# maxgillett/tinysplat

Hardware: AMD Instinct MI355X
Metric: Gaussians*pixels/s fwd+bwd (higher is better)
Workload: dtype f32; 1 GPU; 1000000 random Gaussians, SH degree 3, 1920x1080, fwd+bwd (RGB), BASELINE configs[2]; max_per_tile=614, parallelism=single GPU, tile_lists=16x16 (gsplat's) (auto), gaussian_order=as generated (i.i.d.)

## Files before the change

### include/tinysplat_hip.h

```cpp
#ifndef TINYSPLAT_HIP_H
#define TINYSPLAT_HIP_H

#include <stdint.h>

#ifdef __cplusplus
extern "C" {
#endif

#define TS_ABI_VERSION 8

#define TS_E_BADARG (-1)
#define TS_E_DEGREE (-2)

#define TS_TILE 16
#define TS_SPLAT_RECORD_FLOATS 12
#define TS_PARTIAL_ROW_FLOATS 12

int ts_abi_version(void);

typedef struct ts_camera {
    float fx, fy, cx, cy;
    int32_t img_width, img_height;
    int32_t tile_bounds_x, tile_bounds_y;
    int32_t tile_row0, tile_rows;
// ... 118 lines not shown
#define TS_RASTER_NARROW_WAVES 8
#define TS_RASTER_FLAG_GEN(g) (((g) & 0xff) << 8)
int ts_raster_fwd(int32_t channels, int32_t flags, const ts_camera* cam_host, const int32_t* tile_bins,
                  const int32_t* gaussian_ids_sorted, const float* splats, const float* background,
                  float* out_img, float* final_Ts, int32_t* final_index, uint8_t* clamp_mask,
                  void* stream);
int ts_raster_fwd_planes(int32_t channels, int32_t flags, const ts_camera* cam_host, const int32_t* tile_bins,
                         const int32_t* gaussian_ids_sorted, const float* splats, const float* background,
                         float* out_img, float* out_depth, float* final_Ts, int32_t* final_index,
                         uint8_t* clamp_mask, void* stream);

int ts_raster_fwd_sort(int32_t channels, int32_t flags, const ts_camera* cam_host, const int32_t* tile_bins,
                       const int32_t* bucket_ids, const float* depths, int32_t* gaussian_ids_sorted,
                       const float* splats, const float* background, float* out_img, float* out_depth,
                       float* final_Ts, int32_t* final_index, uint8_t* clamp_mask, void* stream);

int ts_raster_bwd(int32_t channels, int32_t flags, int64_t num_intersects, const ts_camera* cam_host,
                  const int32_t* tile_bins, const int32_t* gaussian_ids_sorted, const float* splats,
                  const float* background, const float* final_Ts, const int32_t* final_index,
                  const float* v_out_img, const float* v_out_alpha, const uint8_t* clamp_mask,
                  float* partials, uint8_t* row_flags, void* stream);
int ts_raster_bwd_planes(int32_t channels, int32_t flags, int64_t num_intersects, const ts_camera* cam_host,
                         const int32_t* tile_bins, const int32_t* gaussian_ids_sorted, const float* splats,
                         const float* background, const float* final_Ts, const int32_t* final_index,
                         const float* v_out_img, const float* v_out_depth, int32_t planes,
                         const float* v_out_alpha, const uint8_t* clamp_mask,
                         float* partials, uint8_t* row_flags, void* stream);

int ts_reduce_partials(int32_t n, int32_t channels, int32_t flags, const int32_t* num_tiles_hit,
                       const int32_t* cum_tiles_hit, const float* partials,
                       const uint8_t* row_flags, const float* splats, float* v_xy, float* v_conic,
                       float* v_colors, float* v_opacity, float* v_depth, const uint8_t* color_mask,
                       void* stream);

#define TS_FRAME_TIGHT 1
#define TS_FRAME_SPLIT 2
#define TS_FRAME_NARROW_WAVES 8
#define TS_FRAME_DIRECT_SCATTER 32
#define TS_FRAME_PLANES 64
#define TS_FRAME_LIST_STATS 256
#define TS_FRAME_SEPARATE_SORT 128
#define TS_FRAME_STRIPE 16
#define TS_FRAME_GROUP_COUNTS 1024
#define TS_FRAME_ONE_WALK 2048
#define TS_FRAME_ROW_SPANS (4096)
#define TS_FRAME_SURVIVORS 512
typedef struct ts_frame {
    int32_t n, num_bases, sh_degree, channels, flags;
    int32_t flag_gen;
    ts_camera cam;
    const float *means, *scales, *quats, *opacities, *colors_dc, *colors_rest;
    const float *view34, *projview, *origin, *background;
    float *xys, *depths, *conics, *colors, *splats;
    int32_t *radii, *num_tiles_hit, *cum_tiles_hit;
    uint8_t* sh_mask;
    int32_t *scan_ws, *bin_ws, *tile_bins;
    int32_t* total_host;
    int64_t num_intersects;
    int64_t capacity;
    int32_t *bucket_ids, *gaussian_ids_sorted;
    float *out_img, *final_Ts;
    int32_t* final_index;
    uint8_t* clamp_mask;
    const float* v_out_img;
    float* partials;
    uint8_t* row_flags;
// ... 361 lines not shown
```

### tinysplat_amd/_lib.py

```python
from __future__ import annotations

import ctypes
import os
from ctypes import POINTER, c_double, c_float, c_int32, c_int64, c_uint32, c_uint64, c_void_p
from pathlib import Path

LIB_PATH = Path(os.environ["TS_LIB_PATH"]) if os.environ.get("TS_LIB_PATH") else \
    Path(__file__).resolve().parent / "csrc" / "libtinysplat_hip.so"
ABI_VERSION = 8
HINT_BALANCED_WALK = 1
HINT_COOP_SPLIT = 1 << 20
RASTER_LOGIT_OPACITY = 1
RASTER_CLAMP_RGB = 2
RASTER_SPLIT_BLOCKS = 4
RASTER_NARROW_WAVES = 8
FRAME_TIGHT = 1
FRAME_SPLIT = 2
FRAME_NARROW_WAVES = 8
FRAME_STRIPE = 16
FRAME_DIRECT_SCATTER = 32
FRAME_PLANES = 64
FRAME_SEPARATE_SORT = 128
FRAME_LIST_STATS = 256
FRAME_SURVIVORS = 512
# ... 114 lines not shown
    "ts_colors_pack_fwd": (c_int32, [c_int32, c_int32, c_int32, _P, _P, _P, _P, _P, _P, c_int32, c_int32,
                                     _P, _P, _P, _P, _P, _CAM, _P, _P, _P]),
    "ts_colors_pack_spans_fwd": (c_int32, [c_int32, c_int32, c_int32, _P, _P, _P, _P, _P, _P, c_int32, c_int32,
                                           _P, _P, _P, _P, _P, _CAM, _P, _P, c_int32, _P, _P]),
    "ts_pack_splats": (c_int32, [c_int32, c_int32, c_int32, _P, _P, _P, _P, _P, _P, _CAM, _P, _P, _P]),
    "ts_raster_fwd": (c_int32, [c_int32, c_int32, _CAM, _P, _P, _P, _P, _P, _P, _P, _P, _P]),
    "ts_raster_bwd": (c_int32, [c_int32, c_int32, c_int64, _CAM, _P, _P, _P, _P, _P, _P, _P, _P, _P, _P, _P, _P]),
    "ts_raster_fwd_planes": (c_int32, [c_int32, c_int32, _CAM, _P, _P, _P, _P, _P, _P, _P, _P, _P, _P]),
    "ts_raster_fwd_sort": (c_int32, [c_int32, c_int32, _CAM, _P, _P, _P, _P, _P, _P, _P, _P, _P, _P, _P, _P]),
    "ts_raster_bwd_planes": (c_int32, [c_int32, c_int32, c_int64, _CAM, _P, _P, _P, _P, _P, _P, _P, _P, c_int32,
                                       _P, _P, _P, _P, _P]),
    "ts_bench_stream_read": (c_int32, [_P, c_int64, _P, _P]),
    "ts_bench_gather48": (c_int32, [_P, _P, c_int64, _P, _P]),
    "ts_photometric_ws_floats": (c_int64, [c_int32, c_int32]),
    "ts_photometric_loss": (c_int32, [c_int32, c_int32, _P, _P, c_float, c_float, _P, _P, _P]),
    "ts_photometric_loss_rgbd": (c_int32, [c_int32, c_int32, c_int32, _P, _P, _P, c_float, c_float, c_float, _P, _P, _P]),
    "ts_photometric_loss_planes": (c_int32, [c_int32, c_int32, _P, _P, _P, _P, c_float, c_float, c_float, _P, _P, _P,
                                             _P]),
    "ts_photometric_loss_reduce": (c_int32, [c_int32, c_int32, c_float, c_float, c_float, _P, _P, _P]),
    "ts_adam_step": (c_int32, [c_int32, _P, _P, _P, _P, _P, _P, _P, c_float, c_float, c_float, _P]),
    "ts_sh_colors_bwd_adam": (c_int32, [c_int32, c_int32, c_int32, _P, _P, _P, _P, _P, _P, _ADAM, _P]),
    "ts_project_bwd_adam": (c_int32, [c_int32, _P, _P, _P, _P, _P, _CAM, c_int32, _P, _P, _P, _P, _P, _P, _ADAM, _P]),
    "ts_frame_bwd_params_adam": (c_int32, [_FRAME, _ADAM, _P]),
    "ts_grad_accum": (c_int32, [c_int32, _P, _P, _P]),
    "ts_densify_classify": (c_int32, [c_int32, _P, _P, _P, POINTER(TsDensifyPolicy), _P, _P]),
    "ts_densify_ws_ints": (c_int64, [c_int32]),
    "ts_densify_plan": (c_int32, [c_int32, _P, _P, _P, _P, _P]),
    "ts_gather_rows": (c_int32, [c_int32, _P, _P, _P, c_int32, c_int32, _P, _P]),
    "ts_split_fixup": (c_int32, [c_int32, _P, _P, _P, _P, _P, _P, _P, _P]),
    "ts_ply_row_floats": (c_int32, [c_int32]),
    "ts_ply_pack_rows": (c_int32, [c_int32, c_int32, _P, _P, _P, _P, _P, _P, _P, _P]),
    "ts_ply_unpack_rows": (c_int32, [c_int32, c_int32, _P, _P, _P, _P, _P, _P, _P, _P]),
    "ts_reduce_partials": (c_int32, [c_int32, c_int32, c_int32, _P, _P, _P, _P, _P, _P, _P, _P, _P, _P, _P, _P]),
    "ts_route_ws_ints": (c_int64, [c_int32, c_int32]),
    "ts_route_count": (c_int32, [c_int32, _P, _P, _CAM, _STRIPES, _P, _P, _P]),
    "ts_route_count_padded": (c_int32, [c_int32, _P, _P, _CAM, _STRIPES, _P, _P, _P, _P]),
    "ts_route_pack": (c_int32, [c_int32, c_int32, _P, _P, _P, _P, _CAM, _STRIPES, _P, _P, _P]),
    "ts_import_records": (c_int32, [c_int32, _P, _CAM, _P, _P, _P, _P, _P]),
    "ts_import_pack": (c_int32, [c_int32, _P, _P, _CAM, _P, _P]),
    "ts_reduce_partials_rows": (c_int32, [c_int32, c_int32, c_int32, _P, _P, _P, _P, _P, _P, _P]),
    "ts_route_accumulate": (c_int32, [c_int32, c_int32, _P, _P, _P, _P, _CAM, _STRIPES, _P, _P, _P, _P, _P, _P, _P, _P]),
    "ts_shard_owner_fwd": (c_int32, [_FRAME, _STRIPES, _P, _P, _P]),
    "ts_shard_owner_fwd_padded": (c_int32, [_FRAME, _STRIPES, _P, _P, _P, _P]),
    "ts_shard_owner_fwd_fused": (c_int32, [c_int32, c_int32, c_int32, _P, _P, _P, _P, _P, _CAM, c_int32, _P, _P, _P, _P,
                                           c_int32, c_int32, _P, _P, _P, _P, _P, _P, _P, _STRIPES, _P, _P, _P, _P]),
    "ts_shard_owner_bwd_fused": (c_int32, [c_int32, c_int32, c_int32, c_int32, _P, _P, _P, _P, _P, _P, _P, _P, _P, _P,
                                           _CAM, _STRIPES, _P, _P, _P, _P, _P, _P, _P, _P, _P, _P, _P, _P, _P]),
    "ts_shard_stripe_fwd_import": (c_int32, [_FRAME, _P, _P]),
    "ts_shard_stripe_bwd": (c_int32, [_FRAME, _P, _P]),
    "ts_shard_owner_bwd": (c_int32, [_FRAME, _STRIPES, _P, _P, _P]),
    "ts_rank_step_struct_bytes": (c_int32, []),
    "ts_shard_rank_fwd_a": (c_int32, [_FRAME, _RANK, _P]),
    "ts_shard_rank_fwd_b": (c_int32, [_FRAME, _RANK, _P]),
    "ts_shard_rank_bwd_a": (c_int32, [_FRAME, _RANK, _P]),
    "ts_shard_rank_bwd_b": (c_int32, [_FRAME, _RANK, _P]),
    "ts_frame_struct_bytes": (c_int32, []),
    "ts_frame_fwd_project": (c_int32, [_FRAME, _P]),
    "ts_frame_fwd_prepare": (c_int32, [_FRAME, _P]),
    "ts_frame_fwd_composite": (c_int32, [_FRAME, _P]),
    "ts_frame_bwd_composite": (c_int32, [_FRAME, _P]),
    "ts_frame_bwd_params": (c_int32, [_FRAME, _P]),
    "ts_set_entry_probe": (c_int32, [_P, _P]),
    "ts_knn_ws_bytes": (c_int64, [c_int32, c_int32, c_int32]),
    "ts_knn": (c_int32, [c_int32, _P, c_int32, _P, c_int32, _P, _P, _P, _P, _P]),
    "ts_init_from_points": (c_int32, [c_int32, c_int32, _P, _P, _P, _P, _P, _P, _P, _P, _P, _P, _P, _P, _P, _P]),
    "ts_opacity_entropy_ws_bytes": (c_int64, [c_int32]),
# ... 129 lines not shown
```

### tinysplat_amd/csrc/frame.hip

```cpp
#include <hip/hip_runtime.h>

#include <atomic>
#include <cstdlib>
#if !defined(TS_NO_ROCTX) && __has_include(<rocprofiler-sdk-roctx/roctx.h>)
#include <rocprofiler-sdk-roctx/roctx.h>
#define TS_HAVE_ROCTX 1
#else
#define TS_HAVE_ROCTX 0
#endif

#include "../../include/tinysplat_hip.h"
#include "raster_survivors.h"

struct TsRange {
#if TS_HAVE_ROCTX
    explicit TsRange(const char* name) { roctxRangePush(name); }
    ~TsRange() { roctxRangePop(); }
#else
    explicit TsRange(const char*) {}
#endif
};

static std::atomic<ts_entry_probe> g_probe{nullptr};
static std::atomic<void*> g_probe_user{nullptr};
// ... 194 lines not shown
                            ts_sort_tiles_stats(num_tiles(f), f->tile_bins, f->depths, f->bucket_ids,
                                                f->gaussian_ids_sorted, f->bin_ws, counter, f->n, f->bin_ws, longest,
                                                stream)));
    }
    if (fused_sort)
        return TS_ENTRY("ts_raster_fwd",
                        ts_surv::raster_fwd_sort(f->channels, raster_flags(f), &f->cam, f->tile_bins, f->bucket_ids,
                                                 f->depths, f->gaussian_ids_sorted, f->splats, f->background,
                                                 f->out_img, planes ? f->out_depth : nullptr, f->final_Ts,
                                                 f->final_index, f->clamp_mask, survivors(f) ? f->survivors : nullptr,
                                                 stream));
    return TS_ENTRY("ts_raster_fwd",
                    ts_raster_fwd_planes(f->channels, raster_flags(f), &f->cam, f->tile_bins, f->gaussian_ids_sorted,
                                         f->splats, f->background, f->out_img, planes ? f->out_depth : nullptr,
                                         f->final_Ts, f->final_index, f->clamp_mask, stream));
}

int ts_frame_bwd_composite(const ts_frame* f, void* stream) {
    TsRange range_("ts_frame_bwd_composite");
    if (bad(f) || f->num_intersects < 0) return TS_E_BADARG;
    const bool planes = (f->flags & TS_FRAME_PLANES) != 0;
    const bool surv = survivors(f);
    TS_TRY(TS_ENTRY("ts_raster_bwd",
                    ts_surv::raster_bwd(f->channels,
                                        ((raster_flags(f) & ~(TS_RASTER_CLAMP_RGB | TS_RASTER_SPLIT_BLOCKS)) | bwd_split(f)) |
                                            TS_RASTER_FLAG_GEN(f->flag_gen),
                                        f->num_intersects, &f->cam, f->tile_bins, f->gaussian_ids_sorted, f->splats,
                                        f->background, f->final_Ts, f->final_index, f->v_out_img,
                                        planes ? f->v_out_depth : nullptr, planes ? 1 : 0, nullptr, f->clamp_mask,
                                        f->partials, f->row_flags, surv ? f->bucket_ids : nullptr,
                                        surv ? f->survivors : nullptr, stream)));
    const bool stripe = (f->flags & TS_FRAME_STRIPE) != 0;
    return TS_ENTRY("ts_reduce_partials",
                    ts_reduce_partials(f->n, f->channels,
                                       TS_RASTER_LOGIT_OPACITY | bwd_split(f) | TS_RASTER_FLAG_GEN(f->flag_gen),
                                       f->num_tiles_hit, f->cum_tiles_hit, f->partials, f->row_flags, f->splats,
                                       f->v_xy, f->v_conic, f->v_colors, f->v_opacity,
                                       f->channels == 4 ? f->v_depth : nullptr, stripe ? f->sh_mask : nullptr, stream));
}

int ts_frame_bwd_params(const ts_frame* f, void* stream) {
    TsRange range_("ts_frame_bwd_params");
    if (bad(f)) return TS_E_BADARG;
    TS_TRY(TS_ENTRY("ts_sh_colors_bwd",
                    ts_sh_colors_bwd(f->n, f->sh_degree, f->num_bases, f->means, f->origin,
                                     (f->flags & TS_FRAME_STRIPE) ? nullptr : f->sh_mask, f->v_colors, f->v_colors_dc,
                                     f->num_bases > 1 ? f->v_colors_rest : nullptr, stream)));
    return TS_ENTRY("ts_project_bwd",
                    ts_project_bwd(f->n, f->means, f->scales, f->quats, f->view34, f->projview, &f->cam, 3, f->radii,
                                   f->v_xy, f->v_depth, f->v_conic, nullptr, f->v_means, f->v_scales, f->v_quats,
                                   stream));
}

int ts_frame_bwd_params_adam(const ts_frame* f, const ts_adam* adam, void* stream) {
    TsRange range_("ts_frame_bwd_params_adam");
    if (bad(f) || !adam) return TS_E_BADARG;
    TS_TRY(TS_ENTRY("ts_sh_colors_bwd_adam",
                    ts_sh_colors_bwd_adam(f->n, f->sh_degree, f->num_bases, f->means, f->origin,
                                          (f->flags & TS_FRAME_STRIPE) ? nullptr : f->sh_mask, f->v_colors,
                                          const_cast<float*>(f->colors_dc),
                                          f->num_bases > 1 ? const_cast<float*>(f->colors_rest) : nullptr, adam,
                                          stream)));
    return TS_ENTRY("ts_project_bwd_adam",
                    ts_project_bwd_adam(f->n, const_cast<float*>(f->means), const_cast<float*>(f->scales),
                                        const_cast<float*>(f->quats), f->view34, f->projview, &f->cam, 3, f->radii,
                                        f->v_xy, f->v_depth, f->v_conic, const_cast<float*>(f->opacities), f->v_opacity,
                                        adam, stream));
}


int ts_shard_owner_fwd(const ts_frame* fo, const ts_stripes* stripes, int32_t* route_ws, int32_t* counts,
// ... 132 lines not shown
```

### tinysplat_amd/csrc/pack.h

```cpp
#pragma once

#include <hip/hip_runtime.h>

#include "../../include/tinysplat_hip.h"
#include "row_spans.h"
#include "splat_math.h"

namespace ts {

struct PackArgs {
    int channels, flags;
    const float* xys;
    const int* radii;
    const float* conics;
    const float* opacity;
    const int* cum_tiles_hit;
    const float* depths;
    float4* splats;
    ts_camera cam;
    int4* row_spans = nullptr;
    int tight = 0;
};

struct PackIn {
    int r;
    float2 xy;
    float op, cxx, cxy, cyy;
};

__device__ __forceinline__ PackIn pack_load(const PackArgs& a, int i) {
    PackIn in;
    in.r = a.radii[i];
    in.xy = reinterpret_cast<const float2*>(a.xys)[i];
    in.op = a.opacity[i];
    in.cxx = a.conics[3 * i]; in.cxy = a.conics[3 * i + 1]; in.cyy = a.conics[3 * i + 2];
    return in;
}
__device__ __forceinline__ float pack_opacity(const PackArgs& a, float op) {
    if (a.flags & TS_RASTER_LOGIT_OPACITY) op = 1.0f / (1.0f + expf(-op));
    return op;
}

__device__ __forceinline__ void store_row_spans(const PackArgs& a, int i, const PackIn& in) {
    const RowSpans s = make_row_spans(a.tight != 0, in.xy.x, in.xy.y, in.op, in.cxx, in.cxy, in.cyy, in.r,
                                      a.cam.tile_bounds_x, a.cam.tile_bounds_y, a.cam.tile_row0, a.cam.tile_rows);
    a.row_spans[i] = make_int4((int)s.w[0], (int)s.w[1], (int)s.w[2], (int)s.w[3]);
}

__device__ __forceinline__ void pack_store(const PackArgs& a, int i, const PackIn& in, float c0, float c1, float c2,
                                           float c3) {
    if (in.r <= 0) return;
    const TileBox b = tile_bbox(in.xy.x, in.xy.y, (float)in.r, a.cam.tile_bounds_x, a.cam.tile_bounds_y,
                                a.cam.tile_row0, a.cam.tile_rows);
    const int w = b.maxx - b.minx, h = b.maxy - b.miny;
    const int cnt = h > 0 ? w * h : 0;
    if (cnt <= 0) return;
    const int excl = a.cum_tiles_hit[i] - cnt;
    const int slot_base = excl - b.miny * w - b.minx;
    a.splats[3 * (size_t)i] = make_float4(in.xy.x, in.xy.y, in.op, in.cxx);
    a.splats[3 * (size_t)i + 1] = make_float4(in.cxy, in.cyy, c0, c1);
    a.splats[3 * (size_t)i + 2] =
        make_float4(c2, c3, __int_as_float(slot_base), __int_as_float(w | (b.minx << 16)));
}

__device__ __forceinline__ void pack_one(const PackArgs& a, int i, float c0, float c1, float c2, float c3) {
    const int r = a.radii[i];
    if (r <= 0) return;
    const float2 xy = reinterpret_cast<const float2*>(a.xys)[i];
    const TileBox b = tile_bbox(xy.x, xy.y, (float)r, a.cam.tile_bounds_x, a.cam.tile_bounds_y,
                                a.cam.tile_row0, a.cam.tile_rows);
    const int w = b.maxx - b.minx, h = b.maxy - b.miny;
    const int cnt = h > 0 ? w * h : 0;
    if (cnt <= 0) return;
    const int excl = a.cum_tiles_hit[i] - cnt;
    const int slot_base = excl - b.miny * w - b.minx;
    float op = a.opacity[i];
    if (a.flags & TS_RASTER_LOGIT_OPACITY) op = 1.0f / (1.0f + expf(-op));
    a.splats[3 * (size_t)i] = make_float4(xy.x, xy.y, op, a.conics[3 * i]);
    a.splats[3 * (size_t)i + 1] = make_float4(a.conics[3 * i + 1], a.conics[3 * i + 2], c0, c1);
    a.splats[3 * (size_t)i + 2] =
        make_float4(c2, c3, __int_as_float(slot_base), __int_as_float(w | (b.minx << 16)));
}

}
```

### tinysplat_amd/csrc/project.hip

```cpp
#include <hip/hip_runtime.h>

#include "../../include/tinysplat_hip.h"
#include "host_util.h"
#include "pack.h"
#include "splat_math.h"
#include "adam_math.h"

namespace {

constexpr int kThreads = 256;
#ifndef TS_SH_THREADS_FWD
#define TS_SH_THREADS_FWD 128
#endif
#ifndef TS_SH_THREADS_BWD
#define TS_SH_THREADS_BWD 256
#endif
typedef float f4v __attribute__((ext_vector_type(4)));
__device__ __forceinline__ void store4(float4* p, float a, float b, float c, float d) {
    f4v v = {a, b, c, d};
    __builtin_nontemporal_store(v, reinterpret_cast<f4v*>(p));
}
constexpr int kShThreadsFwd = TS_SH_THREADS_FWD, kShThreadsBwd = TS_SH_THREADS_BWD;
__device__ __forceinline__ float4 load4_stream(const float4* p) {
    const f4v v = __builtin_nontemporal_load(reinterpret_cast<const f4v*>(p));
// ... 308 lines not shown
    if (pk.row_spans) {
        ts::PackIn in = ts::pack_load(pk, i);
        in.op = ts::pack_opacity(pk, in.op);
        ts::store_row_spans(pk, i, in);
    }
    float Y[KA];
    ts::sh_basis(DEG, means[3 * i] - origin[0], means[3 * i + 1] - origin[1],
                 means[3 * i + 2] - origin[2], Y);
    float c0 = Y[0] * dc[3 * i], c1 = Y[0] * dc[3 * i + 1], c2 = Y[0] * dc[3 * i + 2];
    const float* r = rest + (size_t)i * 3 * (num_bases - 1);
#pragma unroll
    for (int k = 1; k < KA; ++k) {
        c0 = c0 + Y[k] * r[3 * (k - 1)];
        c1 = c1 + Y[k] * r[3 * (k - 1) + 1];
        c2 = c2 + Y[k] * r[3 * (k - 1) + 2];
    }
    c0 = c0 + 0.5f; c1 = c1 + 0.5f; c2 = c2 + 0.5f;
    if (mask) mask[i] = (unsigned char)((c0 >= 0.0f ? 1 : 0) | (c1 >= 0.0f ? 2 : 0) | (c2 >= 0.0f ? 4 : 0));
    c0 = fmaxf(c0, 0.0f); c1 = fmaxf(c1, 0.0f); c2 = fmaxf(c2, 0.0f);
    if (colors) { colors[3 * i] = c0; colors[3 * i + 1] = c1; colors[3 * i + 2] = c2; }
    if (pk.splats) ts::pack_one(pk, i, c0, c1, c2, pk.channels == 4 ? pk.depths[i] : 0.0f);
}

struct ShAdam {
    float *dc, *rest, *m_dc, *v_dc, *m_rest, *v_rest;
    ts::AdamCoef c_dc, c_rest;
};
template <int DEG, bool ADAM>
__global__ __launch_bounds__(kShThreadsBwd) void sh_colors_bwd_kernel(
    int n, int num_bases, const float* __restrict__ means, const float* __restrict__ origin,
    const unsigned char* __restrict__ mask, const float* __restrict__ v_colors,
    float* __restrict__ v_dc, float* __restrict__ v_rest, const ShAdam ad) {
    constexpr int KA = (DEG + 1) * (DEG + 1);
    extern __shared__ __align__(16) float lds[];
    const int RS = 3 * (num_bases - 1);
    const int RSP = RS | 1;
    const int g0 = blockIdx.x * kShThreadsBwd;
    const int cnt = min(kShThreadsBwd, n - g0);
    const int tid = threadIdx.x;
    if (tid < cnt) {
        const int i = g0 + tid;
        float Y[KA];
        ts::sh_basis(DEG, means[3 * i] - origin[0], means[3 * i + 1] - origin[1],
                     means[3 * i + 2] - origin[2], Y);
        const int m = mask ? mask[i] : 7;
        const float v0 = (m & 1) ? v_colors[3 * i] : 0.0f, v1 = (m & 2) ? v_colors[3 * i + 1] : 0.0f,
                    v2 = (m & 4) ? v_colors[3 * i + 2] : 0.0f;
        if (ADAM) {
            const float gd[3] = {Y[0] * v0, Y[0] * v1, Y[0] * v2};
#pragma unroll
            for (int c = 0; c < 3; ++c) {
                float p_ = ad.dc[3 * i + c], m_ = ad.m_dc[3 * i + c], s_ = ad.v_dc[3 * i + c];
                ts::adam_update(p_, gd[c], m_, s_, ad.c_dc);
                ad.dc[3 * i + c] = p_; ad.m_dc[3 * i + c] = m_; ad.v_dc[3 * i + c] = s_;
            }
        } else {
            v_dc[3 * i] = Y[0] * v0; v_dc[3 * i + 1] = Y[0] * v1; v_dc[3 * i + 2] = Y[0] * v2;
        }
        float* r = lds + tid * RSP;
#pragma unroll
        for (int k = 1; k < KA; ++k) {
            r[3 * (k - 1)] = Y[k] * v0; r[3 * (k - 1) + 1] = Y[k] * v1; r[3 * (k - 1) + 2] = Y[k] * v2;
        }
        for (int j = 3 * (KA - 1); j < RS; ++j) r[j] = 0.0f;
    }
    if (RS == 0) return;
    __syncthreads();
    const size_t off = (size_t)g0 * RS;
    float* dst = ADAM ? nullptr : v_rest + off;
    const int total = cnt * RS;
    if ((total & 3) == 0 && ((off) & 3) == 0) {
        float4* dst4 = reinterpret_cast<float4*>(dst);
        for (int f4 = tid; f4 < total / 4; f4 += kShThreadsBwd) {
            float e[4];
#pragma unroll
            for (int u = 0; u < 4; ++u) {
                const int ff = 4 * f4 + u;
                e[u] = lds[(ff / RS) * RSP + (ff % RS)];
            }
            if (ADAM) {
                float4* p4 = reinterpret_cast<float4*>(ad.rest + off) + f4;
                float4* m4 = reinterpret_cast<float4*>(ad.m_rest + off) + f4;
                float4* s4 = reinterpret_cast<float4*>(ad.v_rest + off) + f4;
                float4 pp = *p4, mm = *m4, ss = *s4;
                ts::adam_update(pp.x, e[0], mm.x, ss.x, ad.c_rest); ts::adam_update(pp.y, e[1], mm.y, ss.y, ad.c_rest);
                ts::adam_update(pp.z, e[2], mm.z, ss.z, ad.c_rest); ts::adam_update(pp.w, e[3], mm.w, ss.w, ad.c_rest);
                *p4 = pp; *m4 = mm; *s4 = ss;
            } else {
                store4(dst4 + f4, e[0], e[1], e[2], e[3]);
            }
        }
    } else {
        for (int f = tid; f < total; f += kShThreadsBwd) {
            const float e = lds[(f / RS) * RSP + (f % RS)];
            if (ADAM) {
                float p_ = ad.rest[off + f], m_ = ad.m_rest[off + f], s_ = ad.v_rest[off + f];
                ts::adam_update(p_, e, m_, s_, ad.c_rest);
                ad.rest[off + f] = p_; ad.m_rest[off + f] = m_; ad.v_rest[off + f] = s_;
            } else {
                dst[f] = e;
            }
        }
    }
}
// ... 348 lines not shown
```

### tinysplat_amd/csrc/raster.hip

```cpp
#include <hip/hip_runtime.h>

#include <type_traits>

#include "../../include/tinysplat_hip.h"
#include "host_util.h"
#include "raster_survivors.h"
#include "splat_math.h"

namespace {
#include "sort_network.h"

#ifndef TS_FWD_MIN_WAVES_RGB
#define TS_FWD_MIN_WAVES_RGB 5
#endif
#ifndef TS_FWD_MIN_WAVES_RGBD
#define TS_FWD_MIN_WAVES_RGBD 5
#endif
#ifndef TS_BWD_MIN_WAVES_16
#define TS_BWD_MIN_WAVES_16 5
#endif

#ifndef TS_ABLATE
#define TS_ABLATE 0
#endif

#ifndef TS_STATS
#define TS_STATS 0
#endif
#if TS_STATS
__device__ unsigned long long ts_stats[12];
#define TS_STAT(i, v)                                                                       \
    do {                                                                                    \
        if ((threadIdx.x & 63) == 0) atomicAdd(&ts_stats[i], (unsigned long long)(v));      \
    } while (0)
#else
#define TS_STAT(i, v) ((void)0)
#endif

// ... 1440 lines not shown
        s.mask &= bbox_blocks<WL>(__float_as_int(q2.w), tx);
#pragma unroll
        for (int k = 0; k < NB; ++k)
            if (i > bmax[k]) s.mask &= ~(1 << k);
        const bool keep = (s.mask & ((1 << NB) - 1)) != 0;
        const unsigned long long mask = __ballot(keep);
        const int cnt = __popcll(mask);
        if (keep) {
            const int pos = __popcll(mask & ((1ull << lane) - 1ull));
            const int wm = __float_as_int(q2.w);
            int slot = __float_as_int(q2.z) + ty * (wm & 0xffff) + tx;
            if (SPLIT) slot = 4 * slot + only;
            constexpr int RS = CH == 3 ? 3 : 4;
            lds[RS * pos] = make_float4(s.gx, s.gy, s.hA, s.B);
            lds[RS * pos + 1] = make_float4(s.hC, s.lo, q1.z, q1.w);
            lds[RS * pos + 2] = bwd_record_tail(q2.x, CH == 3 ? __int_as_float(s.mask) : q2.y, i, slot);
            if (CH == 4) lds[RS * pos + 3] = make_float4(__int_as_float(s.mask), 0.f, 0.f, 0.f);
        }
        TS_WAVE_SYNC();
        TS_STAT(2, cnt);
        TS_STAT(7, min(64, hi - sb + 1));
        TS_SEG_ADD(ts_wave_clock_.seg, 0, tseg_p);
        const bool general = __ballot(keep && (s.mask & (1 << NB))) != 0ull;
        if (general)
            bwd_chunk<CH, true>(lds, cnt, fpx, fpy, T, R, vo, fidx, acc, num_isects, partials,
                                     row_flags, lane TS_SEG_ARG);
        else
            bwd_chunk<CH, false>(lds, cnt, fpx, fpy, T, R, vo, fidx, acc, num_isects, partials,
                                      row_flags, lane TS_SEG_ARG);
        TS_WAVE_SYNC();
    }
}

template <int CH>
__global__ __launch_bounds__(256) void reduce_partials_kernel(
    int n, int flags, const int* __restrict__ num_tiles_hit, const int* __restrict__ cum_tiles_hit,
    const float4* __restrict__ partials, const unsigned char* __restrict__ row_flags,
    const float4* __restrict__ splats, float* __restrict__ v_xy, float* __restrict__ v_conic,
    float* __restrict__ v_colors, float* __restrict__ v_opacity, float* __restrict__ v_depth,
    const unsigned char* __restrict__ color_mask, float4* __restrict__ grad_rows) {
    const int i = (int)((long long)blockIdx.x * 256 + threadIdx.x);
    if (i >= n) return;
    const int cnt = num_tiles_hit[i];
    const long long end = cum_tiles_hit[i];
    const unsigned int gen = ((unsigned int)flags >> 8) & 0xffu ? ((unsigned int)flags >> 8) & 0xffu : 1u;
    double s[10];
#pragma unroll
    for (int c = 0; c < 10; ++c) s[c] = 0.0;
    auto add_row = [&](const float4& p0, const float4& p1, const float4& p2) {
        s[0] += (double)p0.x; s[1] += (double)p0.y; s[2] += (double)p0.z; s[3] += (double)p0.w;
        s[4] += (double)p1.x; s[5] += (double)p1.y; s[6] += (double)p1.z; s[7] += (double)p1.w;
        s[8] += (double)p2.x; s[9] += (double)p2.y;
    };
    if (flags & TS_RASTER_SPLIT_BLOCKS) {
        const unsigned int* flags4 = reinterpret_cast<const unsigned int*>(row_flags);
        for (long long sl = end - cnt; sl < end; ++sl) {
            const unsigned int fw = flags4[sl];
            unsigned int f = 0u;
#pragma unroll
            for (int k = 0; k < 4; ++k) f |= (((fw >> (8 * k)) & 0xffu) == gen) ? (0xffu << (8 * k)) : 0u;
            if (f == 0u) continue;
            float4 p0[4], p1[4], p2[4];
#pragma unroll
            for (int k = 0; k < 4; ++k) {
                if (f & (0xffu << (8 * k))) {
                    p0[k] = partials[kRowF4 * (4 * sl + k)]; p1[k] = partials[kRowF4 * (4 * sl + k) + 1];
                    p2[k] = partials[kRowF4 * (4 * sl + k) + 2];
                }
            }
#pragma unroll
            for (int k = 0; k < 4; ++k) {
                if (f & (0xffu << (8 * k))) add_row(p0[k], p1[k], p2[k]);
            }
        }
    } else {
        constexpr int kAhead = TS_REDUCE_AHEAD;
        for (long long s0 = end - cnt; s0 < end; s0 += kAhead) {
            bool f[kAhead];
            float4 p0[kAhead], p1[kAhead], p2[kAhead];
#pragma unroll
            for (int u = 0; u < kAhead; ++u) f[u] = (s0 + u < end) && row_flags[s0 + u] == gen;
#pragma unroll
            for (int u = 0; u < kAhead; ++u) {
                if (f[u]) {
                    p0[u] = partials[kRowF4 * (s0 + u)]; p1[u] = partials[kRowF4 * (s0 + u) + 1];
                    p2[u] = partials[kRowF4 * (s0 + u) + 2];
                }
            }
#pragma unroll
            for (int u = 0; u < kAhead; ++u) {
                if (f[u]) add_row(p0[u], p1[u], p2[u]);
            }
        }
    }
    float4 a0 = make_float4((float)s[0], (float)s[1], (float)s[2], (float)s[3]);
    float4 a1 = make_float4((float)s[4], (float)s[5], (float)s[6], (float)s[7]);
    float4 a2 = make_float4((float)s[8], (float)s[9], 0.f, 0.f);
    float vx = 0.f, vy = 0.f, vop = 0.f;
    if (cnt > 0) {
        const float4 q0 = splats[3 * (size_t)i], q1 = splats[3 * (size_t)i + 1];
        const float A = q0.w, B = q1.x, C = q1.y, op = q0.z;
        vx = A * a0.y + B * a0.z;
        vy = B * a0.y + C * a0.z;
        vop = op > 0.0f ? -a0.x / op : 0.0f;
        if (flags & TS_RASTER_LOGIT_OPACITY) vop *= op * (1.0f - op);
        if (color_mask) {
            const int m = color_mask[i];
            if (!(m & 1)) a1.z = 0.0f;
            if (!(m & 2)) a1.w = 0.0f;
            if (!(m & 4)) a2.x = 0.0f;
        }
    }
    if (grad_rows) {
        grad_rows[3 * (size_t)i] = make_float4(vx, vy, 0.5f * a0.w, a1.x);
        grad_rows[3 * (size_t)i + 1] = make_float4(0.5f * a1.y, a1.z, a1.w, a2.x);
        grad_rows[3 * (size_t)i + 2] = make_float4(CH == 4 ? a2.y : 0.0f, vop, 0.0f, 0.0f);
        return;
    }
    reinterpret_cast<float2*>(v_xy)[i] = make_float2(vx, vy);
    v_opacity[i] = vop;
    v_conic[3 * i] = 0.5f * a0.w; v_conic[3 * i + 1] = a1.x; v_conic[3 * i + 2] = 0.5f * a1.y;
    if (CH == 4 && v_depth == nullptr) {
        reinterpret_cast<float4*>(v_colors)[i] = make_float4(a1.z, a1.w, a2.x, a2.y);
    } else if (CH == 4) {
        v_colors[3 * i] = a1.z; v_colors[3 * i + 1] = a1.w; v_colors[3 * i + 2] = a2.x;
        v_depth[i] = a2.y;
    } else {
        v_colors[3 * i] = a1.z; v_colors[3 * i + 1] = a1.w; v_colors[3 * i + 2] = a2.x;
    }
}

}

extern "C" {
// ... 216 lines not shown
                       final_Ts, final_index, v_out_img, v_out_depth, planes ? 1 : 0, v_out_alpha,  \
                       clamp_mask, partials, row_flags, bucket_ids, sv_meta, sv_cnt)
#define TS_LAUNCH_BWD_X(C, S)                                                                      \
    do {                                                                                           \
        if (narrow) TS_LAUNCH_BWD(C, S, true, false);                                              \
        else if (survivors) TS_LAUNCH_BWD(C, false, false, true);               \
        else TS_LAUNCH_BWD(C, S, false, false);                                                    \
    } while (0)
    if (channels == 3) { if (split) TS_LAUNCH_BWD_X(3, true); else TS_LAUNCH_BWD_X(3, false); }
    else { if (split) TS_LAUNCH_BWD_X(4, true); else TS_LAUNCH_BWD_X(4, false); }
#undef TS_LAUNCH_BWD_X
#undef TS_LAUNCH_BWD
    return launch_status();
}

}

extern "C" {

int ts_reduce_partials(int32_t n, int32_t channels, int32_t flags, const int32_t* num_tiles_hit,
                       const int32_t* cum_tiles_hit, const float* partials,
                       const uint8_t* row_flags, const float* splats, float* v_xy, float* v_conic,
                       float* v_colors, float* v_opacity, float* v_depth, const uint8_t* color_mask,
                       void* stream) {
    if (n < 0 || (channels != 3 && channels != 4)) return TS_E_BADARG;
    if (n == 0) return 0;
    if (!num_tiles_hit || !cum_tiles_hit || !row_flags || !splats || !v_xy || !v_conic || !v_colors || !v_opacity)
        return TS_E_BADARG;
    hipStream_t s = (hipStream_t)stream;
    const float4* pr = reinterpret_cast<const float4*>(partials);
    const float4* sp = reinterpret_cast<const float4*>(splats);
    const int grid = (int)(((long long)n + 255) / 256);
    if (channels == 3)
        hipLaunchKernelGGL(reduce_partials_kernel<3>, dim3(grid), dim3(256), 0, s, n, (int)flags, num_tiles_hit,
                           cum_tiles_hit, pr, row_flags, sp, v_xy, v_conic, v_colors, v_opacity, v_depth, color_mask,
                           (float4*)nullptr);
    else
        hipLaunchKernelGGL(reduce_partials_kernel<4>, dim3(grid), dim3(256), 0, s, n, (int)flags, num_tiles_hit,
                           cum_tiles_hit, pr, row_flags, sp, v_xy, v_conic, v_colors, v_opacity, v_depth, color_mask,
                           (float4*)nullptr);
    return launch_status();
}

int ts_reduce_partials_rows(int32_t n, int32_t channels, int32_t flags, const int32_t* num_tiles_hit,
                            const int32_t* cum_tiles_hit, const float* partials, const uint8_t* row_flags,
                            const float* splats, float* grad_rows, void* stream) {
    if (n < 0 || (channels != 3 && channels != 4)) return TS_E_BADARG;
    if (n == 0) return 0;
    if (!num_tiles_hit || !cum_tiles_hit || !row_flags || !splats || !grad_rows) return TS_E_BADARG;
    hipStream_t s = (hipStream_t)stream;
    const float4* pr = reinterpret_cast<const float4*>(partials);
    const float4* sp = reinterpret_cast<const float4*>(splats);
    float4* gr = reinterpret_cast<float4*>(grad_rows);
    const int grid = (int)(((long long)n + 255) / 256);
    if (channels == 3)
        hipLaunchKernelGGL(reduce_partials_kernel<3>, dim3(grid), dim3(256), 0, s, n, (int)flags, num_tiles_hit,
                           cum_tiles_hit, pr, row_flags, sp, (float*)nullptr, (float*)nullptr, (float*)nullptr,
                           (float*)nullptr, (float*)nullptr, (const unsigned char*)nullptr, gr);
    else
        hipLaunchKernelGGL(reduce_partials_kernel<4>, dim3(grid), dim3(256), 0, s, n, (int)flags, num_tiles_hit,
                           cum_tiles_hit, pr, row_flags, sp, (float*)nullptr, (float*)nullptr, (float*)nullptr,
                           (float*)nullptr, (float*)nullptr, (const unsigned char*)nullptr, gr);
    return launch_status();
}

}
```

### tinysplat_amd/csrc/shard.hip

```cpp
#include <hip/hip_runtime.h>

#include "../../include/tinysplat_hip.h"
#include "host_util.h"
#include "splat_math.h"

namespace {

constexpr int kThreads = 256;
constexpr int kWaves = kThreads / 64;
#include "project_inputs.h"

struct DestRange { int d0, d1; };

__device__ __forceinline__ int stripe_of_row(const ts_stripes& st, int row) {
    int d = 0;
    while (d + 1 < st.num && row >= st.row[d + 1]) ++d;
    return d;
}

__device__ __forceinline__ DestRange dest_range(int i, int n, const float* __restrict__ xys,
                                                const int* __restrict__ radii, const ts_camera& cam,
                                                const ts_stripes& st) {
    DestRange r{1, 0};
    if (i >= n) return r;
    const int rad = radii[i];
    if (rad <= 0) return r;
    const float2 xy = reinterpret_cast<const float2*>(xys)[i];
    const ts::TileBox b = ts::tile_bbox(xy.x, xy.y, (float)rad, cam.tile_bounds_x, cam.tile_bounds_y, 0,
                                        cam.tile_bounds_y);
    if (b.maxx <= b.minx || b.maxy <= b.miny) return r;
    const int lo = max(b.miny, st.row[0]), hi = min(b.maxy, st.row[st.num]);
    if (hi <= lo) return r;
    r.d0 = stripe_of_row(st, lo);
    r.d1 = stripe_of_row(st, hi - 1);
    return r;
}
// ... 38 lines not shown
        const float m[3] = {means3d[3 * i], means3d[3 * i + 1], means3d[3 * i + 2]};
        float sc[3] = {scales[3 * i], scales[3 * i + 1], scales[3 * i + 2]};
        const float4 qv = reinterpret_cast<const float4*>(quats)[i];
        float q[4] = {qv.x, qv.y, qv.z, qv.w};
        prep_inputs(pflags, sc, q, nullptr);
        ts::ProjOut o;
        ts::project_one(C, m, sc, q, o);
        reinterpret_cast<float2*>(xys)[i] = make_float2(o.x, o.y);
        depths[i] = o.depth;
        radii[i] = o.radius;
        conics[3 * i] = o.conic[0]; conics[3 * i + 1] = o.conic[1]; conics[3 * i + 2] = o.conic[2];
        num_tiles_hit[i] = o.tiles;
        if (o.radius > 0) {
            float Y[KA];
            ts::sh_basis(DEG, m[0] - origin[0], m[1] - origin[1], m[2] - origin[2], Y);
            float c0 = Y[0] * dc[3 * i], c1 = Y[0] * dc[3 * i + 1], c2 = Y[0] * dc[3 * i + 2];
            const float* row = rest + (size_t)i * 3 * (num_bases - 1);
#pragma unroll
            for (int k = 1; k < KA; ++k) {
                c0 = c0 + Y[k] * row[3 * (k - 1)];
                c1 = c1 + Y[k] * row[3 * (k - 1) + 1];
                c2 = c2 + Y[k] * row[3 * (k - 1) + 2];
            }
            c0 = c0 + 0.5f; c1 = c1 + 0.5f; c2 = c2 + 0.5f;
            if (mask) mask[i] = (unsigned char)((c0 >= 0.0f ? 1 : 0) | (c1 >= 0.0f ? 2 : 0) | (c2 >= 0.0f ? 4 : 0));
            c0 = fmaxf(c0, 0.0f); c1 = fmaxf(c1, 0.0f); c2 = fmaxf(c2, 0.0f);
            const ts::TileBox b = ts::tile_bbox(o.x, o.y, (float)o.radius, cam.tile_bounds_x, cam.tile_bounds_y,
                                                cam.tile_row0, cam.tile_rows);
            const int w = b.maxx - b.minx, h = b.maxy - b.miny;
            const int cntb = h > 0 ? w * h : 0;
            if (cntb > 0) {
                const int slot_base = (o.tiles - cntb) - b.miny * w - b.minx;
                float op = opacity[i];
                if (rflags & TS_RASTER_LOGIT_OPACITY) op = 1.0f / (1.0f + expf(-op));
                splats[3 * (size_t)i] = make_float4(o.x, o.y, op, o.conic[0]);
                splats[3 * (size_t)i + 1] = make_float4(o.conic[1], o.conic[2], c0, c1);
                splats[3 * (size_t)i + 2] = make_float4(c2, channels == 4 ? o.depth : 0.0f, __int_as_float(slot_base),
                                                        __int_as_float(w | (b.minx << 16)));
            }
            const ts::TileBox fb = ts::tile_bbox(o.x, o.y, (float)o.radius, cam.tile_bounds_x, cam.tile_bounds_y, 0,
                                                 cam.tile_bounds_y);
            if (fb.maxx > fb.minx && fb.maxy > fb.miny) {
                const int lo = max(fb.miny, st.row[0]), hi = min(fb.maxy, st.row[st.num]);
                if (hi > lo) { r.d0 = stripe_of_row(st, lo); r.d1 = stripe_of_row(st, hi - 1); }
            }
        } else if (mask) {
            mask[i] = 0;
        }
    }
    for (int d = 0; d < st.num; ++d) {
        const unsigned long long mm = __ballot(r.d0 <= d && d <= r.d1);
        if (lane == 0) cnt[wave][d] = __popcll(mm);
    }
    __syncthreads();
    if (threadIdx.x < st.num) {
        int sum = 0;
#pragma unroll
        for (int w = 0; w < kWaves; ++w) sum += cnt[w][threadIdx.x];
        block_counts[(size_t)threadIdx.x * gridDim.x + blockIdx.x] = sum;
    }
}

struct GroupBase { int padded; int base[TS_MAX_RANKS + 1]; };
constexpr int kScanThreads = 1024;
__global__ __launch_bounds__(kScanThreads) void route_scan_kernel(int num_blocks, int num_dest,
                                                                  int* __restrict__ block_counts,
                                                                  int* __restrict__ seg,
// ... 423 lines not shown
```

Measured before the change: 2090000 billion Gaussians*pixels/s.

## Read conics/opacities from arrays in reduce; stream SH-rest grads as float4

The frame backward reduce now reads conic and raw opacity from the separate per-Gaussian arrays and recomputes the sigmoid, instead of loading two float4 rows from the packed splat records. The loads are issued early, before the partials accumulation loop. Separately, the SH colors backward kernel gets a fast path for full blocks at the template degree with 16-byte aligned bases, which streams the rest-coefficient gradients (and Adam state) as float4 words with compile-time trip counts. This trades strided 48-byte record reads for narrower array reads and adds code paths with alignment preconditions.

```diff
diff --git a/include/tinysplat_hip.h b/include/tinysplat_hip.h
--- a/include/tinysplat_hip.h
+++ b/include/tinysplat_hip.h
@@ -174,6 +174,11 @@
                        const uint8_t* row_flags, const float* splats, float* v_xy, float* v_conic,
                        float* v_colors, float* v_opacity, float* v_depth, const uint8_t* color_mask,
                        void* stream);
+int ts_reduce_partials_arrays(int32_t n, int32_t channels, int32_t flags, const int32_t* num_tiles_hit,
+                              const int32_t* cum_tiles_hit, const float* partials, const uint8_t* row_flags,
+                              const float* conics, const float* opacities, float* v_xy, float* v_conic,
+                              float* v_colors, float* v_opacity, float* v_depth, const uint8_t* color_mask,
+                              void* stream);
 
 #define TS_FRAME_TIGHT 1
 #define TS_FRAME_SPLIT 2
diff --git a/tinysplat_amd/_lib.py b/tinysplat_amd/_lib.py
--- a/tinysplat_amd/_lib.py
+++ b/tinysplat_amd/_lib.py
@@ -170,6 +170,8 @@
     "ts_ply_pack_rows": (c_int32, [c_int32, c_int32, _P, _P, _P, _P, _P, _P, _P, _P]),
     "ts_ply_unpack_rows": (c_int32, [c_int32, c_int32, _P, _P, _P, _P, _P, _P, _P, _P]),
     "ts_reduce_partials": (c_int32, [c_int32, c_int32, c_int32, _P, _P, _P, _P, _P, _P, _P, _P, _P, _P, _P, _P]),
+    "ts_reduce_partials_arrays": (c_int32, [c_int32, c_int32, c_int32, _P, _P, _P, _P, _P, _P, _P, _P, _P, _P, _P, _P,
+                                            _P]),
     "ts_route_ws_ints": (c_int64, [c_int32, c_int32]),
     "ts_route_count": (c_int32, [c_int32, _P, _P, _CAM, _STRIPES, _P, _P, _P]),
     "ts_route_count_padded": (c_int32, [c_int32, _P, _P, _CAM, _STRIPES, _P, _P, _P, _P]),
diff --git a/tinysplat_amd/csrc/frame.hip b/tinysplat_amd/csrc/frame.hip
--- a/tinysplat_amd/csrc/frame.hip
+++ b/tinysplat_amd/csrc/frame.hip
@@ -250,11 +250,12 @@
                                         surv ? f->survivors : nullptr, stream)));
     const bool stripe = (f->flags & TS_FRAME_STRIPE) != 0;
     return TS_ENTRY("ts_reduce_partials",
-                    ts_reduce_partials(f->n, f->channels,
-                                       TS_RASTER_LOGIT_OPACITY | bwd_split(f) | TS_RASTER_FLAG_GEN(f->flag_gen),
-                                       f->num_tiles_hit, f->cum_tiles_hit, f->partials, f->row_flags, f->splats,
-                                       f->v_xy, f->v_conic, f->v_colors, f->v_opacity,
-                                       f->channels == 4 ? f->v_depth : nullptr, stripe ? f->sh_mask : nullptr, stream));
+                    ts_reduce_partials_arrays(f->n, f->channels,
+                                              TS_RASTER_LOGIT_OPACITY | bwd_split(f) | TS_RASTER_FLAG_GEN(f->flag_gen),
+                                              f->num_tiles_hit, f->cum_tiles_hit, f->partials, f->row_flags, f->conics,
+                                              f->opacities, f->v_xy, f->v_conic, f->v_colors, f->v_opacity,
+                                              f->channels == 4 ? f->v_depth : nullptr, stripe ? f->sh_mask : nullptr,
+                                              stream));
 }
 
 int ts_frame_bwd_params(const ts_frame* f, void* stream) {
diff --git a/tinysplat_amd/csrc/opacity.h b/tinysplat_amd/csrc/opacity.h
--- /dev/null
+++ b/tinysplat_amd/csrc/opacity.h
@@ -0,0 +1,9 @@
+#pragma once
+
+#include <hip/hip_runtime.h>
+
+namespace ts {
+
+__device__ __forceinline__ float opacity_sigmoid(float logit) { return 1.0f / (1.0f + expf(-logit)); }
+
+}
diff --git a/tinysplat_amd/csrc/pack.h b/tinysplat_amd/csrc/pack.h
--- a/tinysplat_amd/csrc/pack.h
+++ b/tinysplat_amd/csrc/pack.h
@@ -3,6 +3,7 @@
 #include <hip/hip_runtime.h>
 
 #include "../../include/tinysplat_hip.h"
+#include "opacity.h"
 #include "row_spans.h"
 #include "splat_math.h"
 
@@ -37,7 +38,7 @@
     return in;
 }
 __device__ __forceinline__ float pack_opacity(const PackArgs& a, float op) {
-    if (a.flags & TS_RASTER_LOGIT_OPACITY) op = 1.0f / (1.0f + expf(-op));
+    if (a.flags & TS_RASTER_LOGIT_OPACITY) op = opacity_sigmoid(op);
     return op;
 }
 
@@ -75,7 +76,7 @@
     const int excl = a.cum_tiles_hit[i] - cnt;
     const int slot_base = excl - b.miny * w - b.minx;
     float op = a.opacity[i];
-    if (a.flags & TS_RASTER_LOGIT_OPACITY) op = 1.0f / (1.0f + expf(-op));
+    if (a.flags & TS_RASTER_LOGIT_OPACITY) op = opacity_sigmoid(op);
     a.splats[3 * (size_t)i] = make_float4(xy.x, xy.y, op, a.conics[3 * i]);
     a.splats[3 * (size_t)i + 1] = make_float4(a.conics[3 * i + 1], a.conics[3 * i + 2], c0, c1);
     a.splats[3 * (size_t)i + 2] =
diff --git a/tinysplat_amd/csrc/project.hip b/tinysplat_amd/csrc/project.hip
--- a/tinysplat_amd/csrc/project.hip
+++ b/tinysplat_amd/csrc/project.hip
@@ -364,12 +364,19 @@
     const unsigned char* __restrict__ mask, const float* __restrict__ v_colors,
     float* __restrict__ v_dc, float* __restrict__ v_rest, const ShAdam ad) {
     constexpr int KA = (DEG + 1) * (DEG + 1);
+    constexpr int RSA = 3 * (KA - 1);
+    constexpr int RSAP = RSA | 1;
     extern __shared__ __align__(16) float lds[];
     const int RS = 3 * (num_bases - 1);
-    const int RSP = RS | 1;
     const int g0 = blockIdx.x * kShThreadsBwd;
     const int cnt = min(kShThreadsBwd, n - g0);
     const int tid = threadIdx.x;
+    __builtin_assume(tid < kShThreadsBwd);
+    const bool base16 = ((ADAM ? (reinterpret_cast<uintptr_t>(ad.rest) | reinterpret_cast<uintptr_t>(ad.m_rest) |
+                                  reinterpret_cast<uintptr_t>(ad.v_rest))
+                               : reinterpret_cast<uintptr_t>(v_rest)) & 15) == 0;
+    const bool streamed = RSA > 0 && num_bases == KA && cnt == kShThreadsBwd && base16;
+    const int RSP = RS | 1;
     if (tid < cnt) {
         const int i = g0 + tid;
         float Y[KA];
@@ -400,8 +407,55 @@
     __syncthreads();
     const size_t off = (size_t)g0 * RS;
     float* dst = ADAM ? nullptr : v_rest + off;
+    if constexpr (RSA > 0) if (streamed) {
+        constexpr int total4 = kShThreadsBwd * RSA / 4;
+        constexpr int per = (total4 + kShThreadsBwd - 1) / kShThreadsBwd;
+        auto word = [&](int f4) {
+            if constexpr (RSAP == RSA) {
+                return reinterpret_cast<const float4*>(lds)[f4];
+            } else {
+                float e[4];
+#pragma unroll
+                for (int c = 0; c < 4; ++c) {
+                    const int ff = 4 * f4 + c;
+                    e[c] = lds[(ff / RSA) * RSAP + (ff % RSA)];
+                }
+                return make_float4(e[0], e[1], e[2], e[3]);
+            }
+        };
+        if (ADAM) {
+            float4* p4 = reinterpret_cast<float4*>(ad.rest + off);
+            float4* m4 = reinterpret_cast<float4*>(ad.m_rest + off);
+            float4* s4 = reinterpret_cast<float4*>(ad.v_rest + off);
+#pragma unroll
+            for (int u = 0; u < per; ++u) {
+                const int f4 = tid + u * kShThreadsBwd;
+                if (f4 < total4) {
+                    const float4 e = word(f4);
+                    float4 pp = p4[f4], mm = m4[f4], ss = s4[f4];
+                    ts::adam_update(pp.x, e.x, mm.x, ss.x, ad.c_rest); ts::adam_update(pp.y, e.y, mm.y, ss.y, ad.c_rest);
+                    ts::adam_update(pp.z, e.z, mm.z, ss.z, ad.c_rest); ts::adam_update(pp.w, e.w, mm.w, ss.w, ad.c_rest);
+                    p4[f4] = pp; m4[f4] = mm; s4[f4] = ss;
+                }
+            }
+        } else {
+            float4* dst4 = reinterpret_cast<float4*>(dst);
+            float4 e[per > 0 ? per : 1];
+#pragma unroll
+            for (int u = 0; u < per; ++u) {
+                const int f4 = tid + u * kShThreadsBwd;
+                e[u] = f4 < total4 ? word(f4) : make_float4(0.f, 0.f, 0.f, 0.f);
+            }
+#pragma unroll
+            for (int u = 0; u < per; ++u) {
+                const int f4 = tid + u * kShThreadsBwd;
+                if (f4 < total4) store4(dst4 + f4, e[u].x, e[u].y, e[u].z, e[u].w);
+            }
+        }
+        return;
+    }
     const int total = cnt * RS;
-    if ((total & 3) == 0 && ((off) & 3) == 0) {
+    if ((total & 3) == 0 && ((off) & 3) == 0 && base16) {
         float4* dst4 = reinterpret_cast<float4*>(dst);
         for (int f4 = tid; f4 < total / 4; f4 += kShThreadsBwd) {
             float e[4];
diff --git a/tinysplat_amd/csrc/raster.hip b/tinysplat_amd/csrc/raster.hip
--- a/tinysplat_amd/csrc/raster.hip
+++ b/tinysplat_amd/csrc/raster.hip
@@ -4,6 +4,7 @@
 
 #include "../../include/tinysplat_hip.h"
 #include "host_util.h"
+#include "opacity.h"
 #include "raster_survivors.h"
 #include "splat_math.h"
 
@@ -1510,17 +1511,20 @@
     }
 }
 
-template <int CH>
+template <int CH, bool ARRAYS>
 __global__ __launch_bounds__(256) void reduce_partials_kernel(
     int n, int flags, const int* __restrict__ num_tiles_hit, const int* __restrict__ cum_tiles_hit,
     const float4* __restrict__ partials, const unsigned char* __restrict__ row_flags,
-    const float4* __restrict__ splats, float* __restrict__ v_xy, float* __restrict__ v_conic,
+    const float4* __restrict__ splats, const float* __restrict__ conics, const float* __restrict__ opacities,
+    float* __restrict__ v_xy, float* __restrict__ v_conic,
     float* __restrict__ v_colors, float* __restrict__ v_opacity, float* __restrict__ v_depth,
     const unsigned char* __restrict__ color_mask, float4* __restrict__ grad_rows) {
     const int i = (int)((long long)blockIdx.x * 256 + threadIdx.x);
     if (i >= n) return;
     const int cnt = num_tiles_hit[i];
     const long long end = cum_tiles_hit[i];
+    float cA = 0.f, cB = 0.f, cC = 0.f, opin = 0.f;
+    if (ARRAYS) { cA = conics[3 * i]; cB = conics[3 * i + 1]; cC = conics[3 * i + 2]; opin = opacities[i]; }
     const unsigned int gen = ((unsigned int)flags >> 8) & 0xffu ? ((unsigned int)flags >> 8) & 0xffu : 1u;
     double s[10];
 #pragma unroll
@@ -1576,8 +1580,14 @@
     float4 a2 = make_float4((float)s[8], (float)s[9], 0.f, 0.f);
     float vx = 0.f, vy = 0.f, vop = 0.f;
     if (cnt > 0) {
-        const float4 q0 = splats[3 * (size_t)i], q1 = splats[3 * (size_t)i + 1];
-        const float A = q0.w, B = q1.x, C = q1.y, op = q0.z;
+        float A, B, C, op;
+        if (ARRAYS) {
+            A = cA; B = cB; C = cC;
+            op = (flags & TS_RASTER_LOGIT_OPACITY) ? ts::opacity_sigmoid(opin) : opin;
+        } else {
+            const float4 q0 = splats[3 * (size_t)i], q1 = splats[3 * (size_t)i + 1];
+            A = q0.w; B = q1.x; C = q1.y; op = q0.z;
+        }
         vx = A * a0.y + B * a0.z;
         vy = B * a0.y + C * a0.z;
         vop = op > 0.0f ? -a0.x / op : 0.0f;
@@ -1860,13 +1870,37 @@
     const float4* sp = reinterpret_cast<const float4*>(splats);
     const int grid = (int)(((long long)n + 255) / 256);
     if (channels == 3)
-        hipLaunchKernelGGL(reduce_partials_kernel<3>, dim3(grid), dim3(256), 0, s, n, (int)flags, num_tiles_hit,
-                           cum_tiles_hit, pr, row_flags, sp, v_xy, v_conic, v_colors, v_opacity, v_depth, color_mask,
-                           (float4*)nullptr);
+        hipLaunchKernelGGL((reduce_partials_kernel<3, false>), dim3(grid), dim3(256), 0, s, n, (int)flags, num_tiles_hit,
+                           cum_tiles_hit, pr, row_flags, sp, (const float*)nullptr, (const float*)nullptr, v_xy, v_conic,
+                           v_colors, v_opacity, v_depth, color_mask, (float4*)nullptr);
     else
-        hipLaunchKernelGGL(reduce_partials_kernel<4>, dim3(grid), dim3(256), 0, s, n, (int)flags, num_tiles_hit,
-                           cum_tiles_hit, pr, row_flags, sp, v_xy, v_conic, v_colors, v_opacity, v_depth, color_mask,
-                           (float4*)nullptr);
+        hipLaunchKernelGGL((reduce_partials_kernel<4, false>), dim3(grid), dim3(256), 0, s, n, (int)flags, num_tiles_hit,
+                           cum_tiles_hit, pr, row_flags, sp, (const float*)nullptr, (const float*)nullptr, v_xy, v_conic,
+                           v_colors, v_opacity, v_depth, color_mask, (float4*)nullptr);
+    return launch_status();
+}
+
+int ts_reduce_partials_arrays(int32_t n, int32_t channels, int32_t flags, const int32_t* num_tiles_hit,
+                              const int32_t* cum_tiles_hit, const float* partials, const uint8_t* row_flags,
+                              const float* conics, const float* opacities, float* v_xy, float* v_conic,
+                              float* v_colors, float* v_opacity, float* v_depth, const uint8_t* color_mask,
+                              void* stream) {
+    if (n < 0 || (channels != 3 && channels != 4)) return TS_E_BADARG;
+    if (n == 0) return 0;
+    if (!num_tiles_hit || !cum_tiles_hit || !row_flags || !conics || !opacities || !v_xy || !v_conic || !v_colors ||
+        !v_opacity)
+        return TS_E_BADARG;
+    hipStream_t s = (hipStream_t)stream;
+    const float4* pr = reinterpret_cast<const float4*>(partials);
+    const int grid = (int)(((long long)n + 255) / 256);
+    if (channels == 3)
+        hipLaunchKernelGGL((reduce_partials_kernel<3, true>), dim3(grid), dim3(256), 0, s, n, (int)flags, num_tiles_hit,
+                           cum_tiles_hit, pr, row_flags, (const float4*)nullptr, conics, opacities, v_xy, v_conic,
+                           v_colors, v_opacity, v_depth, color_mask, (float4*)nullptr);
+    else
+        hipLaunchKernelGGL((reduce_partials_kernel<4, true>), dim3(grid), dim3(256), 0, s, n, (int)flags, num_tiles_hit,
+                           cum_tiles_hit, pr, row_flags, (const float4*)nullptr, conics, opacities, v_xy, v_conic,
+                           v_colors, v_opacity, v_depth, color_mask, (float4*)nullptr);
     return launch_status();
 }
 
@@ -1882,13 +1916,15 @@
     float4* gr = reinterpret_cast<float4*>(grad_rows);
     const int grid = (int)(((long long)n + 255) / 256);
     if (channels == 3)
-        hipLaunchKernelGGL(reduce_partials_kernel<3>, dim3(grid), dim3(256), 0, s, n, (int)flags, num_tiles_hit,
-                           cum_tiles_hit, pr, row_flags, sp, (float*)nullptr, (float*)nullptr, (float*)nullptr,
-                           (float*)nullptr, (float*)nullptr, (const unsigned char*)nullptr, gr);
+        hipLaunchKernelGGL((reduce_partials_kernel<3, false>), dim3(grid), dim3(256), 0, s, n, (int)flags, num_tiles_hit,
+                           cum_tiles_hit, pr, row_flags, sp, (const float*)nullptr, (const float*)nullptr,
+                           (float*)nullptr, (float*)nullptr, (float*)nullptr, (float*)nullptr, (float*)nullptr,
+                           (const unsigned char*)nullptr, gr);
     else
-        hipLaunchKernelGGL(reduce_partials_kernel<4>, dim3(grid), dim3(256), 0, s, n, (int)flags, num_tiles_hit,
-                           cum_tiles_hit, pr, row_flags, sp, (float*)nullptr, (float*)nullptr, (float*)nullptr,
-                           (float*)nullptr, (float*)nullptr, (const unsigned char*)nullptr, gr);
+        hipLaunchKernelGGL((reduce_partials_kernel<4, false>), dim3(grid), dim3(256), 0, s, n, (int)flags, num_tiles_hit,
+                           cum_tiles_hit, pr, row_flags, sp, (const float*)nullptr, (const float*)nullptr,
+                           (float*)nullptr, (float*)nullptr, (float*)nullptr, (float*)nullptr, (float*)nullptr,
+                           (const unsigned char*)nullptr, gr);
     return launch_status();
 }
 
diff --git a/tinysplat_amd/csrc/shard.hip b/tinysplat_amd/csrc/shard.hip
--- a/tinysplat_amd/csrc/shard.hip
+++ b/tinysplat_amd/csrc/shard.hip
@@ -2,6 +2,7 @@
 
 #include "../../include/tinysplat_hip.h"
 #include "host_util.h"
+#include "opacity.h"
 #include "splat_math.h"
 
 namespace {
@@ -106,7 +107,7 @@
             if (cntb > 0) {
                 const int slot_base = (o.tiles - cntb) - b.miny * w - b.minx;
                 float op = opacity[i];
-                if (rflags & TS_RASTER_LOGIT_OPACITY) op = 1.0f / (1.0f + expf(-op));
+                if (rflags & TS_RASTER_LOGIT_OPACITY) op = ts::opacity_sigmoid(op);
                 splats[3 * (size_t)i] = make_float4(o.x, o.y, op, o.conic[0]);
                 splats[3 * (size_t)i + 1] = make_float4(o.conic[1], o.conic[2], c0, c1);
                 splats[3 * (size_t)i + 2] = make_float4(c2, channels == 4 ? o.depth : 0.0f, __int_as_float(slot_base),
```

New measurement: 2100000 billion Gaussians*pixels/s, median of 2. Within noise of the previous version (+0.5%).
